# DIAGNijmegen/bodyct-dram-emph-subtype

Hardware: AMD Instinct MI355X
Metric: CT volumes/sec (train step, 1x128x256x256) (higher is better)
Workload: dtype f32; 1 GPU; BASELINE configs[1]: resnet18segcls train step (fwd+loss+bwd+Adam), batch 2/GPU, 1x128x256x256, fp32, inputs resident in HBM; global_batch=2, parallelism=dp1, hip_graph=False, streams=2

## Files before the change

### bodyct-dram-emph-subtype_amd/csrc/wino_gemm.hip

```cpp
#include <stdlib.h>
#include "wino_gemm.h"

namespace {

template <int MI, int NJ>
__device__ __forceinline__ void zero_acc(f32x16 (&acc)[MI][NJ]) {
#pragma unroll
  for (int mi = 0; mi < MI; ++mi)
#pragma unroll
    for (int nj = 0; nj < NJ; ++nj)
#pragma unroll
      for (int e = 0; e < 16; ++e) acc[mi][nj][e] = 0.f;
}


struct NnTile { const float* Ab; const float* Bb; float* Yb; int mt, nt; };
template <int NJ>
__device__ __forceinline__ NnTile nn_tile(const int idx, const float* A, const float* Bw, float* Y, const int N,
                                          const int K, const int m_tiles, const int n_tiles, const int nblk,
                                          const int npts) {
  constexpr int BN = 64 * NJ;
  const int L = xcd_remap(idx, nblk);
  NnTile t;
  t.nt = L % n_tiles;
  const int r0 = L / n_tiles;
  t.mt = r0 % m_tiles;
  const int xi = r0 / m_tiles;
  t.Ab = A + (((long)t.mt * npts + xi) * 256) * K;
  t.Bb = Bw + ((long)xi * N + (long)t.nt * BN) * K;
  t.Yb = Y + (((long)t.mt * npts + xi) * 256) * N + t.nt * BN;
  return t;
}

template <int NJ>
struct NnLane {
  int tid, lane, wave, li, lh, wm, wn, rsw, a_row, b_row;
  __device__ __forceinline__ NnLane() {
    tid = threadIdx.x;
    lane = tid & 63;
    wave = __builtin_amdgcn_readfirstlane(tid >> 6);
    li = lane & 31; lh = lane >> 5;
    wm = wave & 3; wn = wave >> 2;
    rsw = (li >> 1) & 7;
    a_row = (wm * 64 + li) * 32;
    b_row = 256 * 32 + (wn * NJ * 32 + li) * 32;
  }
};

template <int NJ>
struct NnDma {
  int wave, aoff[4], boff[NJ];
  __device__ __forceinline__ NnDma(const int lane, const int wave_, const int K) : wave(wave_) {
    const int sub = lane >> 3, pslot = lane & 7;
    const int s_even = pslot ^ (lane >> 4), s_odd = s_even ^ 4;
#pragma unroll
    for (int j = 0; j < 4; ++j) aoff[j] = (32 * wave + 8 * j + sub) * K + ((j & 1) ? s_odd : s_even) * 4;
#pragma unroll
    for (int jj = 0; jj < NJ; ++jj) {
      const int nrow = 8 * NJ * wave + 8 * jj + sub;
      boff[jj] = nrow * K + (pslot ^ ((nrow >> 1) & 7)) * 4;
    }
  }
  __device__ __forceinline__ void issue(const float* Ab, const float* Bb, const int it, float* stage) const {
    float* as = stage + 32 * wave * 32;
    float* bs = stage + 256 * 32 + 8 * NJ * wave * 32;
    const float* ag = Ab + it * 32;
    const float* bg = Bb + it * 32;
#pragma unroll
    for (int j = 0; j < 4; ++j)
      __builtin_amdgcn_global_load_lds((const __attribute__((address_space(1))) void*)(ag + aoff[j]),
                                       (__attribute__((address_space(3))) void*)(as + j * 8 * 32), 16, 0, 0);
#pragma unroll
    for (int jj = 0; jj < NJ; ++jj)
      __builtin_amdgcn_global_load_lds((const __attribute__((address_space(1))) void*)(bg + boff[jj]),
                                       (__attribute__((address_space(3))) void*)(bs + jj * 8 * 32), 16, 0, 0);
  }
};

template <int NJ>
__device__ __forceinline__ void nn_kgroups(const float* st, const NnLane<NJ>& ln, f32x16 (&acc)[2][NJ]) {
  f32x4 a0[2], a1[2], bf[2][NJ];
  auto frag = [&](int gk, int buf) __attribute__((always_inline)) {
    const int so = ((2 * gk + ln.lh) ^ ln.rsw) * 4;
    a0[buf] = *reinterpret_cast<const f32x4*>(st + ln.a_row + so);
    a1[buf] = *reinterpret_cast<const f32x4*>(st + ln.a_row + 32 * 32 + so);
#pragma unroll
    for (int nj = 0; nj < NJ; ++nj) bf[buf][nj] = *reinterpret_cast<const f32x4*>(st + ln.b_row + nj * 32 * 32 + so);
  };
  frag(0, 0);
#pragma unroll
  for (int gk = 0; gk < 4; ++gk) {
    if (gk + 1 < 4) frag(gk + 1, (gk + 1) & 1);
#pragma unroll
    for (int e = 0; e < 4; ++e) {
#pragma unroll
      for (int nj = 0; nj < NJ; ++nj) {
        acc[0][nj] = __builtin_amdgcn_mfma_f32_32x32x2f32(a0[gk & 1][e], bf[gk & 1][nj][e], acc[0][nj], 0, 0, 0);
        acc[1][nj] = __builtin_amdgcn_mfma_f32_32x32x2f32(a1[gk & 1][e], bf[gk & 1][nj][e], acc[1][nj], 0, 0, 0);
      }
    }
    if (gk + 1 < 4) __builtin_amdgcn_sched_group_barrier(0x100, 2 + NJ, 0);
    __builtin_amdgcn_sched_group_barrier(0x008, 8 * NJ, 0);
    __builtin_amdgcn_sched_barrier(0);
  }
}

template <int NJ>
__global__ __launch_bounds__(512) void wino_gemm_nn_kernel(const float* __restrict__ A, const float* __restrict__ Bw,
                                                           float* __restrict__ Y, const int Mpad, const int N,
                                                           const int K, const int m_tiles, const int n_tiles,
                                                           const int nblk, const int npts, const GemmEpilogue ep) {
  constexpr int STAGE = (256 + 64 * NJ) * 32;
  __shared__ __attribute__((aligned(1024))) float lds[2 * STAGE];
  const NnLane<NJ> ln;
  const NnTile t = nn_tile<NJ>(blockIdx.x, A, Bw, Y, N, K, m_tiles, n_tiles, nblk, npts);
  const NnDma<NJ> dma(ln.lane, ln.wave, K);
  const int niter = K / 32;
  f32x16 acc[2][NJ];
  zero_acc(acc);

  dma.issue(t.Ab, t.Bb, 0, lds);
  for (int it = 0; it < niter; ++it) {
    __syncthreads();
    if (it + 1 < niter) dma.issue(t.Ab, t.Bb, it + 1, lds + ((it + 1) & 1) * STAGE);
    nn_kgroups<NJ>(lds + (it & 1) * STAGE, ln, acc);
  }

  constexpr int BN = 64 * NJ;
  const bool fused = ep.bias || ep.add || ep.stats;
  constexpr int CW = NJ >= 2 ? 64 : 32;
  constexpr int NR = NJ >= 2 ? NJ / 2 : 1;
  constexpr int P = CW + 8;
  constexpr int Q = CW / 4;
  __syncthreads();
  float* reg = lds + ln.wave * (32 * P);
  const int cq = ln.lane % Q, rs = ln.lane / Q;
  float s1[NR][4], s2[NR][4];
#pragma unroll
  for (int cr = 0; cr < NR; ++cr)
#pragma unroll
    for (int j = 0; j < 4; ++j) { s1[cr][j] = 0.f; s2[cr][j] = 0.f; }
#pragma unroll
  for (int cr = 0; cr < NR; ++cr) {
    const int col = t.nt * BN + ln.wn * NJ * 32 + cr * CW + 4 * cq;
    f32x4 bv = {0.f, 0.f, 0.f, 0.f};
    if (ep.bias) bv = *reinterpret_cast<const f32x4*>(ep.bias + col);
#pragma unroll
    for (int mi = 0; mi < 2; ++mi) {
#pragma unroll
      for (int e = 0; e < 16; ++e)
#pragma unroll
        for (int j = 0; j < CW / 32; ++j)
          reg[((e & 3) + 8 * (e >> 2) + 4 * ln.lh) * P + j * 32 + ln.li] = acc[mi][cr * (CW / 32) + j][e];
#pragma unroll
      for (int r = 0; r < 32 / (64 / Q); ++r) {
        const int row = r * (64 / Q) + rs;
        f32x4 v = *reinterpret_cast<const f32x4*>(reg + row * P + 4 * cq);
        float* o = t.Yb + (long)(ln.wm * 64 + mi * 32 + row) * N + ln.wn * NJ * 32 + cr * CW + 4 * cq;
        if (fused) {
          v += bv;
          if (ep.add) {
            const long oo = o - Y;
            const f32x4 av = *reinterpret_cast<const f32x4*>(ep.add + oo);
            if (ep.gate) {
              const f32x4 gv = *reinterpret_cast<const f32x4*>(ep.gate + oo);
#pragma unroll
              for (int j = 0; j < 4; ++j) v[j] += gv[j] > 0.f ? av[j] : 0.f;
            } else {
              v += av;
            }
          }
#pragma unroll
          for (int j = 0; j < 4; ++j) { s1[cr][j] += v[j]; s2[cr][j] += v[j] * v[j]; }
        }
        *reinterpret_cast<f32x4*>(o) = v;
      }
    }
  }
  if (ep.stats) {
#pragma unroll
    for (int cr = 0; cr < NR; ++cr)
#pragma unroll
      for (int j = 0; j < 4; ++j)
#pragma unroll
        for (int o = Q; o < 64; o <<= 1) {
          s1[cr][j] += __shfl_xor(s1[cr][j], o, 64);
          s2[cr][j] += __shfl_xor(s2[cr][j], o, 64);
        }
    __syncthreads();
    float* red = lds;
    if (rs == 0) {
#pragma unroll
      for (int cr = 0; cr < NR; ++cr)
#pragma unroll
        for (int j = 0; j < 4; ++j) {
          red[(ln.wave * 2 + 0) * 32 * NJ + cr * CW + 4 * cq + j] = s1[cr][j];
          red[(ln.wave * 2 + 1) * 32 * NJ + cr * CW + 4 * cq + j] = s2[cr][j];
        }
    }
    __syncthreads();
    if (ln.tid < 2 * BN) {
      const int which = ln.tid / BN, cc = ln.tid - which * BN;
      const int cwn = cc / (32 * NJ), c2 = cc - cwn * 32 * NJ;
      float v = 0.f;
#pragma unroll
      for (int w = 0; w < 4; ++w) v += red[((cwn * 4 + w) * 2 + which) * 32 * NJ + c2];
      ep.stats[((long)t.mt * 2 + which) * N + t.nt * BN + cc] = v;
    }
  }
}

template <int NJ>
__global__ __launch_bounds__(512) void wino_gemm_nn_pers_kernel(const float* __restrict__ A, const float* __restrict__ Bw,
                                                                float* __restrict__ Y, const int Mpad, const int N,
                                                                const int K, const int m_tiles, const int n_tiles,
                                                                const int nblk, const int npts, const GemmEpilogue ep) {
  constexpr int STAGE = (256 + 64 * NJ) * 32;
  __shared__ __attribute__((aligned(1024))) float s0[STAGE];
  __shared__ __attribute__((aligned(1024))) float s1[STAGE + (NJ == 1 ? 1024 : 0)];
  const NnLane<NJ> ln;
  const NnDma<NJ> dma(ln.lane, ln.wave, K);
  constexpr int BN = 64 * NJ;
  const int niter = K / 32;
  const bool fused = ep.bias || ep.add || ep.stats;
  f32x16 acc[2][NJ];

  int idx = blockIdx.x;
  NnTile cur = nn_tile<NJ>(idx, A, Bw, Y, N, K, m_tiles, n_tiles, nblk, npts);
  dma.issue(cur.Ab, cur.Bb, 0, s0);
  for (;;) {
    const int nxt = idx + gridDim.x;
    const bool more = nxt < nblk;
    NnTile nx = cur;
    if (more) nx = nn_tile<NJ>(nxt, A, Bw, Y, N, K, m_tiles, n_tiles, nblk, npts);
    zero_acc(acc);
    for (int it = 0; it < niter; it += 2) {
      __syncthreads();
      dma.issue(cur.Ab, cur.Bb, it + 1, s1);
      nn_kgroups<NJ>(s0, ln, acc);
      __syncthreads();
      if (it + 2 < niter) dma.issue(cur.Ab, cur.Bb, it + 2, s0);
      else if (more) dma.issue(nx.Ab, nx.Bb, 0, s0);
      nn_kgroups<NJ>(s1, ln, acc);
    }

    constexpr int CW = NJ >= 2 ? 64 : 32;
    constexpr int NR = NJ >= 2 ? NJ / 2 : 1;
    constexpr int P = CW + 8;
    constexpr int Q = CW / 4;
    __syncthreads();
    float* reg = s1 + ln.wave * (16 * P);
    const int cq = ln.lane % Q, rs = ln.lane / Q;
    float s1v[NR][4], s2v[NR][4];
#pragma unroll
    for (int cr = 0; cr < NR; ++cr)
#pragma unroll
      for (int j = 0; j < 4; ++j) { s1v[cr][j] = 0.f; s2v[cr][j] = 0.f; }
#pragma unroll
    for (int cr = 0; cr < NR; ++cr) {
      const int col = cur.nt * BN + ln.wn * NJ * 32 + cr * CW + 4 * cq;
      f32x4 bv = {0.f, 0.f, 0.f, 0.f};
      if (ep.bias) bv = *reinterpret_cast<const f32x4*>(ep.bias + col);
#pragma unroll
      for (int mi = 0; mi < 2; ++mi) {
#pragma unroll
        for (int h = 0; h < 2; ++h) {
#pragma unroll
          for (int e = 8 * h; e < 8 * h + 8; ++e)
#pragma unroll
            for (int j = 0; j < CW / 32; ++j)
              reg[((e & 3) + 8 * ((e >> 2) & 1) + 4 * ln.lh) * P + j * 32 + ln.li] = acc[mi][cr * (CW / 32) + j][e];
#pragma unroll
          for (int r = 0; r < 16 / (64 / Q); ++r) {
            const int row = r * (64 / Q) + rs;
            f32x4 v = *reinterpret_cast<const f32x4*>(reg + row * P + 4 * cq);
            float* o = cur.Yb + (long)(ln.wm * 64 + mi * 32 + 16 * h + row) * N + ln.wn * NJ * 32 + cr * CW + 4 * cq;
            if (fused) {
              v += bv;
              if (ep.add) {
                const long oo = o - Y;
                const f32x4 av = *reinterpret_cast<const f32x4*>(ep.add + oo);
                if (ep.gate) {
                  const f32x4 gv = *reinterpret_cast<const f32x4*>(ep.gate + oo);
#pragma unroll
                  for (int j = 0; j < 4; ++j) v[j] += gv[j] > 0.f ? av[j] : 0.f;
                } else {
                  v += av;
                }
              }
#pragma unroll
              for (int j = 0; j < 4; ++j) { s1v[cr][j] += v[j]; s2v[cr][j] += v[j] * v[j]; }
            }
            *reinterpret_cast<f32x4*>(o) = v;
          }
        }
      }
    }
    if (ep.stats) {
#pragma unroll
      for (int cr = 0; cr < NR; ++cr)
#pragma unroll
        for (int j = 0; j < 4; ++j)
#pragma unroll
          for (int o = Q; o < 64; o <<= 1) {
            s1v[cr][j] += __shfl_xor(s1v[cr][j], o, 64);
            s2v[cr][j] += __shfl_xor(s2v[cr][j], o, 64);
          }
      __syncthreads();
      float* red = s1;
      if (rs == 0) {
#pragma unroll
        for (int cr = 0; cr < NR; ++cr)
#pragma unroll
          for (int j = 0; j < 4; ++j) {
            red[(ln.wave * 2 + 0) * 32 * NJ + cr * CW + 4 * cq + j] = s1v[cr][j];
            red[(ln.wave * 2 + 1) * 32 * NJ + cr * CW + 4 * cq + j] = s2v[cr][j];
          }
      }
      __syncthreads();
      if (ln.tid < 2 * BN) {
        const int which = ln.tid / BN, cc = ln.tid - which * BN;
        const int cwn = cc / (32 * NJ), c2 = cc - cwn * 32 * NJ;
        float v = 0.f;
#pragma unroll
        for (int w = 0; w < 4; ++w) v += red[((cwn * 4 + w) * 2 + which) * 32 * NJ + c2];
        ep.stats[((long)cur.mt * 2 + which) * N + cur.nt * BN + cc] = v;
      }
    }
    if (!more) break;
    idx = nxt;
    cur = nx;
  }
}
#ifndef DRAM_STREAM_NT
#define DRAM_STREAM_NT 2
#endif
template <int NJ, int KT, int S, bool DB = false, int KH = 1>
__global__ __launch_bounds__(256, DB ? 2 : 1) void wino_gemm_nn_stream_kernel(const float* __restrict__ A,
                                                                    const float* __restrict__ Bw, float* __restrict__ Y,
                                                                    const int npts, const int m64, const int per_wg,
                                                                    const int total) {
  constexpr int N = 64 * NJ;
  constexpr int STG = 64 * KT;
  constexpr int SPR = KT / 4;
  constexpr int RPI = 64 / SPR;
  constexpr int IPW = 64 / RPI / 4;
  constexpr int BPW = N / RPI / 4;
  constexpr int KG = KT / 8;
  constexpr int P = DB ? 40 : 32 * NJ + 8;
  constexpr int KS = KT * KH;
  static_assert(S == 3 || S == 4, "ring depth");
  static_assert(KH == 1 || (KH == 2 && DB && S == 3), "k halves: direct-B form, three stages");
  __shared__ __attribute__((aligned(1024))) float st0[STG], st1[STG], st2[STG], st3[S == 4 ? STG : 64];
  __shared__ __attribute__((aligned(1024))) float bt[DB ? 64 : N * KT];
  __shared__ __attribute__((aligned(16))) float turn[4 * 32 * P];

  const int tid = threadIdx.x, lane = tid & 63;
  const int wave = __builtin_amdgcn_readfirstlane(tid >> 6);
  const int li = lane & 31, lh = lane >> 5;
  const int i0 = blockIdx.x * per_wg;
  const int n = (i0 + per_wg <= total ? per_wg : total - i0);
  if (n <= 0) return;

  int aoff[IPW], boff[BPW];
#pragma unroll
  for (int j = 0; j < IPW; ++j) {
    const int row = RPI * (wave + 4 * j) + lane / SPR, ph = lane % SPR;
    aoff[j] = row * KS + ((ph & ~15) | ((ph ^ row) & 15)) * 4;
  }
#pragma unroll
  for (int j = 0; j < BPW; ++j) {
    const int row = RPI * (wave + 4 * j) + lane / SPR, ph = lane % SPR;
    boff[j] = row * KT + ((ph & ~15) | ((ph ^ row) & 15)) * 4;
  }
  auto a_src = [&](int item) __attribute__((always_inline)) {
    const int ti = item / KH, h = item - ti * KH;
    const int xi = ti / m64, t = ti - xi * m64;
    return A + (((long)(t >> 2) * npts + xi) * 256 + (t & 3) * 64) * KS + h * KT;
  };
  auto issue_a = [&](int item, float* stage) __attribute__((always_inline)) {
    const float* src = a_src(item);
#pragma unroll
    for (int j = 0; j < IPW; ++j)
      __builtin_amdgcn_global_load_lds((const __attribute__((address_space(1))) void*)(src + aoff[j]),
                                       (__attribute__((address_space(3))) void*)(stage + (wave + 4 * j) * 256), 16, 0,
                                       DRAM_STREAM_NT);
  };
  auto stage_of = [&](int k) __attribute__((always_inline)) -> float* {
    return k == 0 ? st0 : (k == 1 ? st1 : (k == 2 ? st2 : st3));
  };

  const int r0 = 32 * (wave & 1), c0 = 32 * NJ * (wave >> 1);
  const int arow = r0 + li;
  f32x4 bfr[NJ][KG * KH];
  auto load_b = [&](int xi) __attribute__((always_inline)) {
    if (DB) {
      const float* srcd = Bw + (long)xi * N * KS;
#pragma unroll
      for (int nj = 0; nj < NJ; ++nj)
#pragma unroll
        for (int kg = 0; kg < KG * KH; ++kg)
          bfr[nj][kg] = *reinterpret_cast<const f32x4*>(srcd + (c0 + nj * 32 + li) * KS + (2 * kg + lh) * 4);
      __builtin_amdgcn_s_waitcnt(0x0F70);
      asm volatile("" ::: "memory");
      return;
    }
    __syncthreads();
    const float* src = Bw + (long)xi * N * KT;
#pragma unroll
    for (int j = 0; j < BPW; ++j)
      __builtin_amdgcn_global_load_lds((const __attribute__((address_space(1))) void*)(src + boff[j]),
                                       (__attribute__((address_space(3))) void*)(bt + (wave + 4 * j) * 256), 16, 0, 0);
    __builtin_amdgcn_s_waitcnt(0x0F70);
    asm volatile("" ::: "memory");
    __syncthreads();
#pragma unroll
    for (int nj = 0; nj < NJ; ++nj) {
      const int brow = c0 + nj * 32 + li;
#pragma unroll
      for (int kg = 0; kg < KG; ++kg) {
        const int sl = 2 * kg + lh;
        bfr[nj][kg] = *reinterpret_cast<const f32x4*>(bt + brow * KT + ((sl & ~15) | ((sl ^ brow) & 15)) * 4);
      }
    }
  };

  int xi_cur = i0 / KH / m64;
#pragma unroll
  for (int k = 0; k < S - 1; ++k)
    if (k < n) issue_a(i0 + k, stage_of(k));
  load_b(xi_cur);

  float* reg = turn + wave * (32 * P);
  constexpr int Q = 8 * NJ;
  const int cq = lane % Q, rs = lane / Q;

  constexpr int U = S * KH;
  f32x16 acc[NJ];
  for (int itb = 0; itb < n; itb += U) {
#pragma unroll
    for (int k = 0; k < U; ++k) {
      const int it = itb + k;
      const int h = k % KH;
      if (it < n) {
        const int item = i0 + it;
        const int ti = item / KH;
        const int xi = ti / m64, t = ti - xi * m64;
        if (h == 0 && xi != xi_cur) {
          xi_cur = xi;
          load_b(xi);
        }
        if (it + S - 2 < n) __builtin_amdgcn_s_waitcnt(0x0F70 | ((IPW * (S - 2)) & 15) | (((IPW * (S - 2)) >> 4) << 14));
        else __builtin_amdgcn_s_waitcnt(0x0F70);
        asm volatile("" ::: "memory");
        __builtin_amdgcn_s_barrier();
        if (it + S - 1 < n) issue_a(item + S - 1, stage_of((k + S - 1) % S));
        const float* stg = stage_of(k % S);
        if (h == 0) {
#pragma unroll
          for (int nj = 0; nj < NJ; ++nj)
#pragma unroll
            for (int e = 0; e < 16; ++e) acc[nj][e] = 0.f;
        }
#pragma unroll
        for (int kg = 0; kg < KG; ++kg) {
          const int sl = 2 * kg + lh;
          const f32x4 af = *reinterpret_cast<const f32x4*>(stg + arow * KT + ((sl & ~15) | ((sl ^ arow) & 15)) * 4);
#pragma unroll
          for (int e = 0; e < 4; ++e)
#pragma unroll
            for (int nj = 0; nj < NJ; ++nj)
              acc[nj] = __builtin_amdgcn_mfma_f32_32x32x2f32(af[e], bfr[nj][h * KG + kg][e], acc[nj], 0, 0, 0);
        }
        if (h != KH - 1) continue;
        float* yb = Y + (((long)(t >> 2) * npts + xi) * 256 + (t & 3) * 64 + r0) * N + c0;
        if (DB) {
          const int cq8 = lane & 7, rs8 = lane >> 3;
#pragma unroll
          for (int nj = 0; nj < NJ; ++nj) {
#pragma unroll
            for (int e = 0; e < 16; ++e) reg[((e & 3) + 8 * (e >> 2) + 4 * lh) * P + li] = acc[nj][e];
#pragma unroll
            for (int r = 0; r < 4; ++r) {
              const int row = r * 8 + rs8;
              *reinterpret_cast<f32x4*>(yb + (long)row * N + nj * 32 + 4 * cq8) =
                  *reinterpret_cast<const f32x4*>(reg + row * P + 4 * cq8);
            }
          }
        } else {
#pragma unroll
          for (int e = 0; e < 16; ++e)
#pragma unroll
            for (int nj = 0; nj < NJ; ++nj) reg[((e & 3) + 8 * (e >> 2) + 4 * lh) * P + nj * 32 + li] = acc[nj][e];
#pragma unroll
          for (int r = 0; r < Q / 2; ++r) {
            const int row = r * (64 / Q) + rs;
            *reinterpret_cast<f32x4*>(yb + (long)row * N + 4 * cq) = *reinterpret_cast<const f32x4*>(reg + row * P + 4 * cq);
          }
        }
      }
    }
  }
}

typedef __bf16 bf16x8 __attribute__((ext_vector_type(8)));

template <int NJ, int NT>
__global__ __launch_bounds__(512) void wino_gemm_nn_bf16_kernel(const float* __restrict__ A, const float* __restrict__ Bw,
                                                                float* __restrict__ Y, const int Mpad, const int N,
                                                                const int K, const int m_tiles, const int n_tiles,
                                                                const int nblk, const int npts) {
  constexpr int STAGE = (256 + 64 * NJ) * 32;
  __shared__ __attribute__((aligned(1024))) float lds[2 * STAGE];
  const int tid = threadIdx.x;
  const int lane = tid & 63;
  const int wave = __builtin_amdgcn_readfirstlane(tid >> 6);
  const NnTile t = nn_tile<NJ>(blockIdx.x, A, Bw, Y, N, K, m_tiles, n_tiles, nblk, npts);
  const NnDma<NJ> dma(lane, wave, K);
  const int niter = K / 32;
  f32x16 acc[2][NJ];
  zero_acc(acc);

  const int li = lane & 31, lh = lane >> 5;
  const int wm = wave & 3, wn = wave >> 2;
  const int rsw = (li >> 1) & 7;
  const int a_row = (wm * 64 + li) * 32;
  const int b_row = 256 * 32 + (wn * NJ * 32 + li) * 32;

  dma.issue(t.Ab, t.Bb, 0, lds);
  for (int it = 0; it < niter; ++it) {
    __syncthreads();
    if (it + 1 < niter) dma.issue(t.Ab, t.Bb, it + 1, lds + ((it + 1) & 1) * STAGE);
    const float* st = lds + (it & 1) * STAGE;
#pragma unroll
    for (int j = 0; j < 2; ++j) {
      const int sh = ((2 * j + lh) ^ rsw) * 4, sl = ((4 + 2 * j + lh) ^ rsw) * 4;
      bf16x8 ah[2], al[2], bh[NJ], bl[NJ];
#pragma unroll
      for (int mi = 0; mi < 2; ++mi) {
        ah[mi] = *reinterpret_cast<const bf16x8*>(st + a_row + mi * 32 * 32 + sh);
        if (NT > 1) al[mi] = *reinterpret_cast<const bf16x8*>(st + a_row + mi * 32 * 32 + sl);
      }
#pragma unroll
      for (int nj = 0; nj < NJ; ++nj) {
        bh[nj] = *reinterpret_cast<const bf16x8*>(st + b_row + nj * 32 * 32 + sh);
        if (NT > 1) bl[nj] = *reinterpret_cast<const bf16x8*>(st + b_row + nj * 32 * 32 + sl);
      }
#pragma unroll
      for (int nj = 0; nj < NJ; ++nj)
#pragma unroll
        for (int mi = 0; mi < 2; ++mi) {
          if (NT > 1) {
            acc[mi][nj] = __builtin_amdgcn_mfma_f32_32x32x16_bf16(al[mi], bh[nj], acc[mi][nj], 0, 0, 0);
            acc[mi][nj] = __builtin_amdgcn_mfma_f32_32x32x16_bf16(ah[mi], bl[nj], acc[mi][nj], 0, 0, 0);
          }
          acc[mi][nj] = __builtin_amdgcn_mfma_f32_32x32x16_bf16(ah[mi], bh[nj], acc[mi][nj], 0, 0, 0);
        }
    }
  }

#pragma unroll
  for (int mi = 0; mi < 2; ++mi)
#pragma unroll
    for (int e = 0; e < 16; ++e) {
      const int row = wm * 64 + mi * 32 + (e & 3) + 8 * (e >> 2) + 4 * lh;
      float* o = t.Yb + (long)row * N + wn * NJ * 32 + li;
#pragma unroll
      for (int nj = 0; nj < NJ; ++nj) o[nj * 32] = acc[mi][nj][e];
    }
}

struct TnTile {
  int nt, mt, split, xi;
  int t0, t1;
  __device__ __forceinline__ long row(const int it, const int npts) const {
    const int tt = t0 + it * 32;
    return ((long)(tt >> 8) * npts + xi) * 256 + (tt & 255);
  }
};
__device__ __forceinline__ TnTile tn_item(int L, const int m_tiles, const int n_tiles, const int nsplit, const int kper,
                                          const int Tpad) {
  TnTile t;
  t.nt = L % n_tiles; L /= n_tiles;
  t.mt = L % m_tiles; L /= m_tiles;
  t.split = L % nsplit;
  t.xi = L / nsplit;
  t.t0 = t.split * kper;
  t.t1 = (t.t0 + kper < Tpad) ? t.t0 + kper : Tpad;
  return t;
}
__device__ __forceinline__ TnTile tn_tile(const int bid, const int nblk, const int m_tiles, const int n_tiles,
                                          const int nsplit, const int kper, const int Tpad) {
  return tn_item(xcd_remap(bid, nblk), m_tiles, n_tiles, nsplit, kper, Tpad);
}
template <int WMW, int MI, int NJ>
__global__ __launch_bounds__(512) void wino_gemm_tn_kernel(const float* __restrict__ Ah, const float* __restrict__ Bh,
                                                           float* __restrict__ slab, const int Tpad, const int M,
                                                           const int N, const int m_tiles, const int n_tiles,
                                                           const int nsplit, const int kper, const int nblk,
                                                           const int npts) {
  constexpr int WNW = 8 / WMW;
  constexpr int BM = WMW * 32 * MI, BN = WNW * 32 * NJ;
  static_assert(BM % 64 == 0 && BM <= 256 && BN % 64 == 0 && BN <= 256, "one DMA piece = 256 floats");
  constexpr int STAGE = 32 * (BM + BN);
  constexpr int AQ = BM / 4, ARPP = 64 / AQ, APW = BM / 64;
  constexpr int BQ = BN / 4, BRPP = 64 / BQ, BPW = BN / 64;
  __shared__ __attribute__((aligned(1024))) float lds[2 * STAGE];

  const int tid = threadIdx.x;
  const int lane = tid & 63;
  const int wave = __builtin_amdgcn_readfirstlane(tid >> 6);
  const TnTile t = tn_tile(blockIdx.x, nblk, m_tiles, n_tiles, nsplit, kper, Tpad);
  int bcol = t.nt * BN + (lane % BQ) * 4;
  if (bcol > N - 4) bcol = N - 4;
  const float* Ab = Ah + (long)(lane / AQ) * M + t.mt * BM + (lane % AQ) * 4;
  const float* Bb = Bh + (long)(lane / BQ) * N + bcol;

  auto issue = [&](int it, int stage) __attribute__((always_inline)) {
    float* as = lds + stage * STAGE;
    float* bs = as + 32 * BM;
    const long row = t.row(it, npts);
    const float* ag = Ab + row * M;
    const float* bg = Bb + row * N;
#pragma unroll
    for (int j = 0; j < APW; ++j) {
      const int p = APW * wave + j;
      __builtin_amdgcn_global_load_lds((const __attribute__((address_space(1))) void*)(ag + (long)(p * ARPP) * M),
                                       (__attribute__((address_space(3))) void*)(as + p * 256), 16, 0, 0);
    }
#pragma unroll
    for (int jj = 0; jj < BPW; ++jj) {
      const int p = BPW * wave + jj;
      __builtin_amdgcn_global_load_lds((const __attribute__((address_space(1))) void*)(bg + (long)(p * BRPP) * N),
                                       (__attribute__((address_space(3))) void*)(bs + p * 256), 16, 0, 0);
    }
  };
// ... 272 lines not shown
      else __builtin_amdgcn_s_waitcnt(0x0F70);
      asm volatile("" ::: "memory");
      __builtin_amdgcn_s_barrier();
      if (full || it + S - 1 < n) issue(it + S - 1, a_of((k + S - 1) % S), b_of((k + S - 1) % S));
      const float* as = a_of(k) + wm * 32 + li;
      const float* bs = b_of(k) + wn * 64 + li;
#pragma unroll
      for (int kk = 0; kk < R / 2; ++kk) {
        const int kr = 2 * kk + lh;
        const float af = as[kr * M], b0 = bs[kr * N], b1 = bs[kr * N + 32];
        acc[0] = __builtin_amdgcn_mfma_f32_32x32x2f32(af, b0, acc[0], 0, 0, 0);
        acc[1] = __builtin_amdgcn_mfma_f32_32x32x2f32(af, b1, acc[1], 0, 0, 0);
      }
    };
    int itb = 0;
    for (; itb + 2 * S - 2 < n; itb += S) {
#pragma unroll
      for (int k = 0; k < S; ++k) stage(k, itb + k, true);
    }
    for (; itb < n; itb += S) {
#pragma unroll
      for (int k = 0; k < S; ++k)
        if (itb + k < n) stage(k, itb + k, false);
    }

    float* sb = slab + (((long)split * npts + xi) * M) * N;
#pragma unroll
    for (int e = 0; e < 16; ++e) {
      const int row = wm * 32 + (e & 3) + 8 * (e >> 2) + 4 * lh;
      float* o = sb + (long)row * N + wn * 64 + li;
      o[0] = acc[0][e];
      o[32] = acc[1][e];
    }
  }
}

typedef short s16x4 __attribute__((ext_vector_type(4)));
typedef short s16x8 __attribute__((ext_vector_type(8)));

template <int WMW, int MI, int NJ, int NT>
__global__ __launch_bounds__(512) void wino_gemm_tn_bf16_kernel(const float* __restrict__ Ah, const float* __restrict__ Bh,
                                                                float* __restrict__ slab, const int Tpad, const int M,
                                                                const int N, const int m_tiles, const int n_tiles,
                                                                const int nsplit, const int kper, const int nblk,
                                                                const int npts) {
  constexpr int WNW = 8 / WMW;
  constexpr int BM = WMW * 32 * MI, BN = WNW * 32 * NJ;
  static_assert(BM % 64 == 0 && BM <= 256 && BN % 64 == 0 && BN <= 256, "one DMA piece = 256 floats");
  constexpr int STAGE = 32 * (BM + BN);
  constexpr int AQ = BM / 4, ARPP = 64 / AQ, APW = BM / 64;
  constexpr int BQ = BN / 4, BRPP = 64 / BQ, BPW = BN / 64;
  __shared__ __attribute__((aligned(1024))) float lds[2 * STAGE];

  const int tid = threadIdx.x;
  const int lane = tid & 63;
  const int wave = __builtin_amdgcn_readfirstlane(tid >> 6);
  const TnTile t = tn_tile(blockIdx.x, nblk, m_tiles, n_tiles, nsplit, kper, Tpad);

  int acol[APW], bcol[BPW];
#pragma unroll
  for (int j = 0; j < APW; ++j) {
    const int r3 = (j * ARPP + lane / AQ) & 3, slot = lane % AQ;
    acol[j] = t.mt * BM + ((((slot >> 2) ^ r3) << 2) | (slot & 3)) * 4;
  }
#pragma unroll
  for (int j = 0; j < BPW; ++j) {
    const int r3 = (j * BRPP + lane / BQ) & 3, slot = lane % BQ;
    int c = t.nt * BN + ((((slot >> 2) ^ r3) << 2) | (slot & 3)) * 4;
    bcol[j] = c > N - 4 ? N - 4 : c;
  }
  const float* Ab = Ah + (long)(lane / AQ) * M;
  const float* Bb = Bh + (long)(lane / BQ) * N;

  auto issue = [&](int it, int stage) __attribute__((always_inline)) {
    float* as = lds + stage * STAGE;
    float* bs = as + 32 * BM;
    const long row = t.row(it, npts);
    const float* ag = Ab + row * M;
    const float* bg = Bb + row * N;
#pragma unroll
    for (int j = 0; j < APW; ++j) {
      const int p = APW * wave + j;
      __builtin_amdgcn_global_load_lds((const __attribute__((address_space(1))) void*)(ag + (long)(p * ARPP) * M + acol[j]),
                                       (__attribute__((address_space(3))) void*)(as + p * 256), 16, 0, 0);
    }
#pragma unroll
    for (int jj = 0; jj < BPW; ++jj) {
      const int p = BPW * wave + jj;
      __builtin_amdgcn_global_load_lds((const __attribute__((address_space(1))) void*)(bg + (long)(p * BRPP) * N + bcol[jj]),
                                       (__attribute__((address_space(3))) void*)(bs + p * 256), 16, 0, 0);
    }
  };

  f32x16 acc[MI][NJ];
  zero_acc(acc);

  const int li = lane & 31, lh = lane >> 5;
  const int wm = wave % WMW, wn = wave / WMW;
  const int niter = (t.t1 - t.t0) / 32;

  const int g4 = lane >> 4, q = (lane >> 2) & 3, p4 = lane & 3;
  const int rrow = (g4 >> 1) * 8 + q;
  const int cbyte = (g4 & 1) * 32 + p4 * 8;
  int a_hi[MI], a_lo[MI], b_hi[NJ], b_lo[NJ];
#pragma unroll
  for (int mi = 0; mi < MI; ++mi) {
    const int ch = 2 * (wm * MI + mi);
    a_hi[mi] = rrow * BM * 4 + ((ch ^ q) * 64) + cbyte;
    a_lo[mi] = rrow * BM * 4 + (((ch + 1) ^ q) * 64) + cbyte;
  }
#pragma unroll
  for (int nj = 0; nj < NJ; ++nj) {
    const int ch = 2 * (wn * NJ + nj);
    b_hi[nj] = 32 * BM * 4 + rrow * BN * 4 + ((ch ^ q) * 64) + cbyte;
    b_lo[nj] = 32 * BM * 4 + rrow * BN * 4 + (((ch + 1) ^ q) * 64) + cbyte;
  }
  auto frag = [&](const char* st, int off, int rstride) __attribute__((always_inline)) {
    const s16x4 r0 = __builtin_amdgcn_ds_read_tr16_b64_v4i16((__attribute__((address_space(3))) s16x4*)(st + off));
    const s16x4 r1 =
        __builtin_amdgcn_ds_read_tr16_b64_v4i16((__attribute__((address_space(3))) s16x4*)(st + off + 4 * rstride));
    return __builtin_bit_cast(bf16x8, __builtin_shufflevector(r0, r1, 0, 1, 2, 3, 4, 5, 6, 7));
  };

  if (niter > 0) issue(0, 0);
  for (int it = 0; it < niter; ++it) {
    __syncthreads();
    if (it + 1 < niter) issue(it + 1, (it + 1) & 1);
    const char* st = reinterpret_cast<const char*>(lds + (it & 1) * STAGE);
#pragma unroll
    for (int s16 = 0; s16 < 2; ++s16) {
      bf16x8 ah[MI], al[MI], bh[NJ], bl[NJ];
#pragma unroll
      for (int mi = 0; mi < MI; ++mi) {
        ah[mi] = frag(st, a_hi[mi] + s16 * 16 * BM * 4, BM * 4);
        if (NT > 1) al[mi] = frag(st, a_lo[mi] + s16 * 16 * BM * 4, BM * 4);
      }
#pragma unroll
      for (int nj = 0; nj < NJ; ++nj) {
        bh[nj] = frag(st, b_hi[nj] + s16 * 16 * BN * 4, BN * 4);
        if (NT > 1) bl[nj] = frag(st, b_lo[nj] + s16 * 16 * BN * 4, BN * 4);
      }
#pragma unroll
      for (int nj = 0; nj < NJ; ++nj)
#pragma unroll
        for (int mi = 0; mi < MI; ++mi) {
          if (NT > 1) {
            acc[mi][nj] = __builtin_amdgcn_mfma_f32_32x32x16_bf16(al[mi], bh[nj], acc[mi][nj], 0, 0, 0);
            acc[mi][nj] = __builtin_amdgcn_mfma_f32_32x32x16_bf16(ah[mi], bl[nj], acc[mi][nj], 0, 0, 0);
          }
          acc[mi][nj] = __builtin_amdgcn_mfma_f32_32x32x16_bf16(ah[mi], bh[nj], acc[mi][nj], 0, 0, 0);
        }
    }
  }

  float* sb = slab + (((long)t.split * npts + t.xi) * M + t.mt * BM) * N + t.nt * BN;
#pragma unroll
  for (int mi = 0; mi < MI; ++mi)
#pragma unroll
    for (int e = 0; e < 16; ++e) {
      const int row = wm * 32 * MI + mi * 32 + (e & 3) + 8 * (e >> 2) + 4 * lh;
      float* o = sb + (long)row * N + wn * 32 * NJ + li;
#pragma unroll
      for (int nj = 0; nj < NJ; ++nj)
        if (t.nt * BN + wn * 32 * NJ + nj * 32 + li < N) o[nj * 32] = acc[mi][nj][e];
    }
}

__global__ __launch_bounds__(256) void slab_sum_kernel(const float* __restrict__ slab, float* __restrict__ out, const long n,
                                                       const int nsplit) {
  __shared__ float part[4][64];
  const int r = threadIdx.x & 63, kg = threadIdx.x >> 6;
  for (long i0 = blockIdx.x * 64L; i0 < n; i0 += (long)gridDim.x * 64L) {
    const long i = i0 + r;
    const bool live = i < n;
    float p[8];
#pragma unroll
    for (int j = 0; j < 8; ++j) p[j] = 0.f;
    if (live) {
      int k = kg;
      for (; k + 28 < nsplit; k += 32) {
#pragma unroll
        for (int j = 0; j < 8; ++j) p[j] += slab[(long)(k + 4 * j) * n + i];
      }
      for (int j = 0; k < nsplit; k += 4, ++j) p[j] += slab[(long)k * n + i];
    }
    part[kg][r] = ((p[0] + p[1]) + (p[2] + p[3])) + ((p[4] + p[5]) + (p[6] + p[7]));
    __syncthreads();
    if (kg == 0 && live) out[i] = (part[0][r] + part[1][r]) + (part[2][r] + part[3][r]);
    __syncthreads();
  }
}
}


bool plan_tn(const DramConvDesc* d, const WinoGeom& g, TnPlan& p) {
  const int M = d->Cout, N = d->Cin;
  p.bm = M % 256 == 0 ? 256 : (M % 128 == 0 ? 128 : 64);
  const int ncand = p.bm == 256 ? 3 : 2;
  const int cand[3] = {256, 128, 64};
  p.bn = 0;
  int best_pad = 1 << 30;
  for (int i = 0; i < ncand; ++i) {
    const int padded = (N + cand[i] - 1) / cand[i] * cand[i];
    if (padded * 100 <= N * 113) { p.bn = cand[i]; break; }
    if (padded < best_pad) { best_pad = padded; p.bn = cand[i]; }
  }
  p.m_tiles = M / p.bm;
  p.n_tiles = (N + p.bn - 1) / p.bn;
  if (p.bn >= 128 && (p.bn > 128 || p.bm == 256)) {
    const long w1 = (long)g.npts * p.m_tiles * p.n_tiles;
    const int hb = p.bn / 2, hn = (N + hb - 1) / hb;
    const long w2 = (long)g.npts * p.m_tiles * hn;
    if (w1 >= 512 && (double)((w2 + 255) / 256) * 0.5 * 1.03 < (double)((w1 + 255) / 256)) {
      p.bn = hb;
      p.n_tiles = hn;
    }
  }
  const int base = g.npts * p.m_tiles * p.n_tiles;
  const int k32 = g.Tpad / 32;
  int ns = 1;
  while (base * ns < (g.npts == 1 ? 256 : 512) && ns * 2 <= k32 / 4 && ns < (g.npts == 1 ? 256 : 16)) ns *= 2;
  p.nsplit = ns;
  p.kper = ((k32 + ns - 1) / ns) * 32;
  return true;
}

int run_nn(const float* A, const float* U, float* Y, const WinoGeom& g, int N, int K, hipStream_t s,
           const GemmEpilogue ep, const int math, const bool alone) {
  const int m_tiles = g.Tpad / 256;
  int nj = 1;
  double best = 1e30;
  for (int c = 4; c >= 1; c >>= 1) {
    if (N % (64 * c) != 0) continue;
    const long wgs = (long)g.npts * m_tiles * (N / (64 * c));
    const double cost = (double)((wgs + 255) / 256) * c * (c == 4 ? 1.0 : (c == 2 ? 1.03 : 1.10));
    if (cost < best) { best = cost; nj = c; }
  }
  const int n_tiles = N / (64 * nj);
  const int nblk = g.npts * m_tiles * n_tiles;
  DramProf prof(DRAM_FAM_WINO_GEMM_NN, nj, 2.0 * g.npts * (double)g.Tpad * N * K,
                4.0 * g.npts * ((double)g.Tpad * (K + N) + (double)N * K), s,
                g.npts > 1 ? 2.0 * g.B * g.D * g.H * g.W * (double)N * K * 27.0 : -1.0);
  if (math) {
#define WNB(NJ_, NT_)                                                                                                  \
  hipLaunchKernelGGL((wino_gemm_nn_bf16_kernel<NJ_, NT_>), dim3(nblk), dim3(512), 0, s, A, U, Y, g.Tpad, N, K, m_tiles, \
                     n_tiles, nblk, g.npts)
    if (math == 1) { if (nj == 4) WNB(4, 3); else if (nj == 2) WNB(2, 3); else WNB(1, 3); }
    else { if (nj == 4) WNB(4, 1); else if (nj == 2) WNB(2, 1); else WNB(1, 1); }
#undef WNB
    DRAM_LAUNCH_CHECK();
    return DRAM_OK;
  }
#define WNN(NJ_)                                                                                                   \
  hipLaunchKernelGGL((wino_gemm_nn_kernel<NJ_>), dim3(nblk), dim3(512), 0, s, A, U, Y, g.Tpad, N, K, m_tiles, n_tiles, \
                     nblk, g.npts, ep)
  const char* se = tune_env("DRAM_NN_STREAM");
  const int stream_on = se ? atoi(se) : 1;
  const bool fused = ep.bias || ep.add || ep.gate || ep.stats;
  if (stream_on && !fused && g.npts > 1 && g.Tpad % 256 == 0 &&
      ((N == 64 && (K == 128 || K == 64)) || (N == 128 && K == 64))) {
    const int m64 = g.Tpad / 64;
    const long total = (long)g.npts * m64;
    if (total < (1L << 31) && (total >= 4096 || stream_on == 2)) {
      const int wgs = stream_on == 2 ? 8 : 256;
      const int per_wg = (int)((total + wgs - 1) / wgs);
      const int grid = (int)((total + per_wg - 1) / per_wg);
#define WNS(NJ_, KT_, S_)                                                                                          \
  hipLaunchKernelGGL((wino_gemm_nn_stream_kernel<NJ_, KT_, S_>), dim3(grid), dim3(256), 0, s, A, U, Y, g.npts, m64, \
                     per_wg, (int)total)
      const char* sde = tune_env("DRAM_NN_STREAM_DB");
      const int sdb = sde ? atoi(sde) : (alone ? 7 : 0);
      const int wgs2 = stream_on == 2 ? 8 : 512;
      const int per2 = (int)((total + wgs2 - 1) / wgs2);
      const int grid2 = (int)((total + per2 - 1) / per2);
      if (N == 64 && K == 128 && (sdb & 4)) {
        const long total2 = 2 * total;
        if (total2 < (1L << 31)) {
          const int perk = 2 * (int)((total + wgs2 - 1) / wgs2);
          const int gridk = (int)((total2 + perk - 1) / perk);
          hipLaunchKernelGGL((wino_gemm_nn_stream_kernel<1, 64, 3, true, 2>), dim3(gridk), dim3(256), 0, s, A, U, Y, g.npts,
                             m64, perk, (int)total2);
        } else WNS(1, 128, 3);
      }
      else if (N == 64 && K == 128) WNS(1, 128, 3);
      else if (N == 64 && (sdb & 1))
        hipLaunchKernelGGL((wino_gemm_nn_stream_kernel<1, 64, 3, true>), dim3(grid2), dim3(256), 0, s, A, U, Y, g.npts, m64,
                           per2, (int)total);
      else if (N == 128 && (sdb & 2))
        hipLaunchKernelGGL((wino_gemm_nn_stream_kernel<2, 64, 3, true>), dim3(grid2), dim3(256), 0, s, A, U, Y, g.npts, m64,
                           per2, (int)total);
      else if (N == 64) WNS(1, 64, 4);
      else WNS(2, 64, 4);
#undef WNS
      DRAM_LAUNCH_CHECK();
      return DRAM_OK;
    }
  }
  const char* pe = tune_env("DRAM_NN_PERSIST");
  const int persist = pe ? atoi(pe) : 1;
  if (persist && !fused && nj <= 2 && (K / 32) % 2 == 0) {
    const int rounds = (nblk + 255) / 256;
    int grid = ((nblk + rounds - 1) / rounds + 7) / 8 * 8;
    if (grid > 256) grid = 256;
    if (grid > nblk) grid = nblk;
#define WNP(NJ_)                                                                                                   \
  hipLaunchKernelGGL((wino_gemm_nn_pers_kernel<NJ_>), dim3(grid), dim3(512), 0, s, A, U, Y, g.Tpad, N, K, m_tiles, \
                     n_tiles, nblk, g.npts, ep)
    if (nj == 2) WNP(2);
    else WNP(1);
#undef WNP
    DRAM_LAUNCH_CHECK();
    return DRAM_OK;
  }
  if (nj == 4) WNN(4);
  else if (nj == 2) WNN(2);
  else WNN(1);
#undef WNN
  DRAM_LAUNCH_CHECK();
  return DRAM_OK;
}

int run_tn(const float* Ah, const float* Bh, float* slab, const WinoGeom& g, const TnPlan& p, const int M, const int N,
           const int math, hipStream_t s) {
  const int nblk = g.npts * p.nsplit * p.m_tiles * p.n_tiles;
  DramProf prof(DRAM_FAM_WINO_GEMM_TN, p.bm * 1000 + p.bn, 2.0 * g.npts * (double)g.Tpad * M * N,
                4.0 * g.npts * ((double)g.Tpad * (M + N) + (double)p.nsplit * M * N), s,
                g.npts > 1 ? 2.0 * g.B * g.D * g.H * g.W * (double)M * N * 27.0 : -1.0);
  auto launch = [&](auto kernel) {
    hipLaunchKernelGGL(kernel, dim3(nblk), dim3(512), 0, s, Ah, Bh, slab, g.Tpad, M, N, p.m_tiles, p.n_tiles, p.nsplit,
                       p.kper, nblk, g.npts);
  };
#define WTN(WM_, MI_, NJ_)                                             \
  launch(math == 1   ? wino_gemm_tn_bf16_kernel<WM_, MI_, NJ_, 3>      \
         : math == 2 ? wino_gemm_tn_bf16_kernel<WM_, MI_, NJ_, 1>      \
                     : wino_gemm_tn_kernel<WM_, MI_, NJ_>)
  const char* te = tune_env("DRAM_NN_STREAM");
  const int tn_stream = te ? atoi(te) : 1;
  if (math == 0 && tn_stream) {
    const bool t64 = g.npts > 1 && M == 64 && N == 64 && p.kper % 64 == 0 && g.Tpad % 64 == 0;
    if (g.npts > 1 && M == 64 && N == 128 && p.bm == 64 && p.bn == 128) {
      const int nchains = g.npts * p.nsplit;
      const int grid = tn_stream == 2 && nchains > 8 ? 8 : nchains;
      hipLaunchKernelGGL((wino_gemm_tn_stream_kernel<3>), dim3(grid), dim3(256), 0, s, Ah, Bh, slab, g.Tpad, p.nsplit, p.kper,
                         nchains, g.npts);
      DRAM_LAUNCH_CHECK();
      return DRAM_OK;
    }
    const int niter = p.kper / 32;
    const bool whole = niter % 2 == 0 && (long)p.kper * p.nsplit == g.Tpad;
    if (!t64 && whole && (tn_stream == 2 || (g.npts > 1 && niter <= 4))) {
      const int slots = 256 * (p.bm + p.bn <= 256 ? 2 : 1);
      const int rounds = (nblk + slots - 1) / slots;
      int grid = ((nblk + rounds - 1) / rounds + 7) / 8 * 8;
      if (grid > slots) grid = slots;
      if (tn_stream == 2) grid = 8;
      if (grid > nblk) grid = nblk;
      const int per_wg = (nblk + grid - 1) / grid;
      grid = (nblk + per_wg - 1) / per_wg;
      if (per_wg > 1 || tn_stream == 2) {
#define WTP(WM_, MI_, NJ_)                                                                                              \
  hipLaunchKernelGGL((wino_gemm_tn_pers_kernel<WM_, MI_, NJ_>), dim3(grid), dim3(512), 0, s, Ah, Bh, slab, g.Tpad, M, N, \
                     p.m_tiles, p.n_tiles, p.nsplit, p.kper, nblk, g.npts, per_wg)
        if (p.bm == 256 && p.bn == 256) WTP(4, 2, 4);
        else if (p.bm == 256 && p.bn == 128) WTP(4, 2, 2);
        else if (p.bm == 256 && p.bn == 64) WTP(4, 2, 1);
        else if (p.bm == 128 && p.bn == 256) WTP(2, 2, 2);
        else if (p.bm == 128 && p.bn == 128) WTP(2, 2, 1);
        else if (p.bm == 64 && p.bn == 256) WTP(2, 1, 2);
        else if (p.bm == 64 && p.bn == 128) WTP(2, 1, 1);
        else return DRAM_ERR_UNSUPPORTED;
#undef WTP
        DRAM_LAUNCH_CHECK();
        return DRAM_OK;
      }
    }
  }
  if (math == 0 && g.npts > 1 && M == 64 && N == 64 && p.kper % 64 == 0 && g.Tpad % 64 == 0)
    hipLaunchKernelGGL(wino_gemm_tn64_kernel, dim3(g.npts * p.nsplit), dim3(512), 0, s, Ah, Bh, slab, g.Tpad, p.nsplit,
                       p.kper, g.npts * p.nsplit, g.npts);
  else if (p.bm == 256 && p.bn == 256) WTN(4, 2, 4);
  else if (p.bm == 256 && p.bn == 128) WTN(4, 2, 2);
  else if (p.bm == 256 && p.bn == 64) WTN(4, 2, 1);
  else if (p.bm == 128 && p.bn == 256) WTN(2, 2, 2);
  else if (p.bm == 128 && p.bn == 128) WTN(2, 2, 1);
  else if (p.bm == 64 && p.bn == 256) WTN(2, 1, 2);
  else if (p.bm == 64 && p.bn == 128) WTN(2, 1, 1);
  else return DRAM_ERR_UNSUPPORTED;
#undef WTN
  DRAM_LAUNCH_CHECK();
  return DRAM_OK;
}

namespace {
bool c1_ok(const DramConvDesc* d) {
  if (!d || d->k != 1 || d->stride != 1 || d->pad != 0) return false;
  if (d->B < 1 || d->D < 1 || d->H < 1 || d->W < 1) return false;
  if (d->Do != d->D || d->Ho != d->H || d->Wo != d->W) return false;
  if (d->Cin < 64 || d->Cout < 64 || d->Cin % 64 != 0 || d->Cout % 64 != 0) return false;
  const long long M = (long long)d->B * d->D * d->H * d->W;
  const long long cmax = d->Cin > d->Cout ? d->Cin : d->Cout;
  return M % 256 == 0 && M * cmax < (1LL << 31);
}
WinoGeom c1_geom(const DramConvDesc* d) {
  WinoGeom g{};
  g.B = d->B; g.D = d->D; g.H = d->H; g.W = d->W; g.d = 1;
  g.nz = g.ny = g.nx = 1;
  g.npts = 1;
  g.T = g.Tpad = d->B * d->D * d->H * d->W;
  return g;
}
}

extern "C" int dram_conv1x1_applicable(const DramConvDesc* d) { return c1_ok(d) ? 1 : 0; }

extern "C" int dram_conv1x1_num_stat_rows(const DramConvDesc* d) {
  if (!c1_ok(d)) return DRAM_ERR_UNSUPPORTED;
  return c1_geom(d).Tpad / 256;
}

extern "C" int dram_conv1x1_fwd(const float* x, const float* w2d, const float* bias, float* y, float* stats_partial,
                                const DramConvDesc* d, dram_stream_t stream) {
  if (!x || !w2d || !y) return DRAM_ERR_BAD_ARG;
  if (!c1_ok(d)) return DRAM_ERR_UNSUPPORTED;
  return run_nn(x, w2d, y, c1_geom(d), d->Cout, d->Cin, (hipStream_t)stream,
                GemmEpilogue{bias, nullptr, nullptr, stats_partial});
}

extern "C" int dram_conv1x1_bwd_data(const float* dy, const float* wt, float* dx, const float* add, const float* gate,
                                     const DramConvDesc* d, dram_stream_t stream) {
  if (!dy || !wt || !dx || (gate && !add)) return DRAM_ERR_BAD_ARG;
  if (!c1_ok(d)) return DRAM_ERR_UNSUPPORTED;
  return run_nn(dy, wt, dx, c1_geom(d), d->Cin, d->Cout, (hipStream_t)stream, GemmEpilogue{nullptr, add, gate, nullptr});
}

extern "C" size_t dram_conv1x1_bwd_weight_workspace(const DramConvDesc* d) {
  if (!c1_ok(d)) return 0;
  TnPlan p;
  plan_tn(d, c1_geom(d), p);
  return (size_t)p.nsplit * d->Cout * d->Cin * sizeof(float);
}

extern "C" int dram_conv1x1_bwd_weight(const float* x, const float* dy, float* dw, const DramConvDesc* d, void* workspace,
                                       size_t workspace_bytes, dram_stream_t stream) {
  if (!x || !dy || !dw) return DRAM_ERR_BAD_ARG;
  if (!c1_ok(d)) return DRAM_ERR_UNSUPPORTED;
  const WinoGeom g = c1_geom(d);
  TnPlan p;
  plan_tn(d, g, p);
  const size_t need = (size_t)p.nsplit * d->Cout * d->Cin * sizeof(float);
  if (p.nsplit > 1 && (!workspace || workspace_bytes < need)) return DRAM_ERR_WORKSPACE;
  hipStream_t s = (hipStream_t)stream;
  float* slab = p.nsplit > 1 ? (float*)workspace : dw;
  const int rc = run_tn(dy, x, slab, g, p, d->Cout, d->Cin, 0, s);
  if (rc != DRAM_OK) return rc;
  if (p.nsplit > 1) {
    const long n = (long)d->Cout * d->Cin;
    const int grid = (int)((n + 63) / 64 > 4096 ? 4096 : (n + 63) / 64);
    DramProf prof(DRAM_FAM_WINO_WGRAD_OUT, 0, 0.0, 4.0 * (double)n * (p.nsplit + 1), s);
    hipLaunchKernelGGL(slab_sum_kernel, dim3(grid), dim3(256), 0, s, slab, dw, n, p.nsplit);
    DRAM_LAUNCH_CHECK();
  }
  return DRAM_OK;
}
```

Measured before the change: 56.00 volumes/sec.

## Overlap persistent NN GEMM epilogue stores with next tile's MFMA main loop

Adds a persistent Winograd NN GEMM kernel that keeps two accumulator sets and drains the previous tile's results through a per-wave LDS transpose buffer, interleaved into the first k-groups of the next tile using sched_group_barrier. The aim is to hide epilogue store latency behind MFMA work instead of stalling at the end of each tile. It becomes the default for the persistent, non-fused path (persist=3 restores the old kernel). It drops the fused stats epilogue from this path and doubles accumulator registers, which risks register pressure. There is also a debug grid=7 option.

```diff
diff --git a/bodyct-dram-emph-subtype_amd/csrc/wino_gemm.hip b/bodyct-dram-emph-subtype_amd/csrc/wino_gemm.hip
--- a/bodyct-dram-emph-subtype_amd/csrc/wino_gemm.hip
+++ b/bodyct-dram-emph-subtype_amd/csrc/wino_gemm.hip
@@ -1,4 +1,5 @@
 #include <stdlib.h>
+#include <type_traits>
 #include "wino_gemm.h"
 
 namespace {
@@ -332,6 +333,214 @@
     cur = nx;
   }
 }
+
+template <int NJ>
+struct NnTurn {
+  static constexpr int CW = 32 * NJ;
+  static constexpr int P = CW + 8;
+  static constexpr int Q = CW / 4;
+  static constexpr int RPR = 64 / Q;
+  static constexpr int NRD = 16 / RPR;
+  static constexpr int NWR = 8 * NJ;
+  float* reg;
+  float* po;
+  int N, cq, rs;
+  template <int T>
+  __device__ __forceinline__ void write(const NnLane<NJ>& ln, const f32x16 (&prev)[2][NJ]) const {
+#pragma unroll
+    for (int e = 8 * (T & 1); e < 8 * (T & 1) + 8; ++e)
+#pragma unroll
+      for (int j = 0; j < NJ; ++j)
+        reg[((e & 3) + 8 * ((e >> 2) & 1) + 4 * ln.lh) * P + j * 32 + ln.li] = prev[T >> 1][j][e];
+  }
+  __device__ __forceinline__ void read(f32x4 (&v)[NRD]) const {
+#pragma unroll
+    for (int r = 0; r < NRD; ++r) v[r] = *reinterpret_cast<const f32x4*>(reg + (r * RPR + rs) * P + 4 * cq);
+  }
+  template <int T>
+  __device__ __forceinline__ void store(const f32x4 (&v)[NRD]) const {
+#pragma unroll
+    for (int r = 0; r < NRD; ++r)
+      *reinterpret_cast<f32x4*>(po + (long)((T >> 1) * 32 + (T & 1) * 16 + r * RPR) * N) = v[r];
+  }
+  __device__ __forceinline__ void all(const NnLane<NJ>& ln, const f32x16 (&prev)[2][NJ]) const {
+    f32x4 v[NRD];
+    write<0>(ln, prev); read(v); store<0>(v);
+    write<1>(ln, prev); read(v); store<1>(v);
+    write<2>(ln, prev); read(v); store<2>(v);
+    write<3>(ln, prev); read(v); store<3>(v);
+  }
+};
+
+template <int NJ, int T0, int NT>
+__device__ __forceinline__ void nn_kgroups_drain(const float* st, const NnLane<NJ>& ln, f32x16 (&acc)[2][NJ],
+                                                 const f32x16 (&prev)[2][NJ], const NnTurn<NJ>& tr) {
+  using TR = NnTurn<NJ>;
+  f32x4 a0[2], a1[2], bf[2][NJ];
+  f32x4 va[TR::NRD], vb[TR::NRD];
+  auto frag = [&](int gk, int buf) __attribute__((always_inline)) {
+    const int so = ((2 * gk + ln.lh) ^ ln.rsw) * 4;
+    a0[buf] = *reinterpret_cast<const f32x4*>(st + ln.a_row + so);
+    a1[buf] = *reinterpret_cast<const f32x4*>(st + ln.a_row + 32 * 32 + so);
+#pragma unroll
+    for (int nj = 0; nj < NJ; ++nj) bf[buf][nj] = *reinterpret_cast<const f32x4*>(st + ln.b_row + nj * 32 * 32 + so);
+  };
+  frag(0, 0);
+  auto region = [&](auto gkc) __attribute__((always_inline)) {
+    constexpr int gk = decltype(gkc)::value;
+    if (gk + 1 < 4) frag(gk + 1, (gk + 1) & 1);
+    if constexpr (NT == 1) {
+      if (gk == 0) { tr.template write<T0>(ln, prev); tr.read(va); }
+      if (gk == 1) tr.template store<T0>(va);
+    } else {
+      if (gk == 0) tr.template write<T0>(ln, prev);
+      if (gk == 1) { tr.read(va); tr.template write<T0 + NT - 1>(ln, prev); }
+      if (gk == 2) { tr.template store<T0>(va); tr.read(vb); }
+      if (gk == 3) tr.template store<T0 + NT - 1>(vb);
+    }
+#pragma unroll
+    for (int e = 0; e < 4; ++e) {
+#pragma unroll
+      for (int nj = 0; nj < NJ; ++nj) {
+        acc[0][nj] = __builtin_amdgcn_mfma_f32_32x32x2f32(a0[gk & 1][e], bf[gk & 1][nj][e], acc[0][nj], 0, 0, 0);
+        acc[1][nj] = __builtin_amdgcn_mfma_f32_32x32x2f32(a1[gk & 1][e], bf[gk & 1][nj][e], acc[1][nj], 0, 0, 0);
+      }
+    }
+    constexpr bool rd = NT == 2 && (gk == 1 || gk == 2);
+    constexpr bool wr = (gk == 0) || (gk == 1 && NT == 2);
+    constexpr bool stg = NT == 2 ? (gk == 2 || gk == 3) : gk == 1;
+    constexpr int nrd = (gk + 1 < 4 ? 2 + NJ : 0) + (rd ? TR::NRD : 0);
+    if constexpr (nrd > 0) __builtin_amdgcn_sched_group_barrier(0x100, nrd, 0);
+    if constexpr (wr && NT == 1) {
+#pragma unroll
+      for (int i = 0; i < 4; ++i) {
+        __builtin_amdgcn_sched_group_barrier(0x008, 1, 0);
+        __builtin_amdgcn_sched_group_barrier(0x200, 2, 0);
+      }
+      __builtin_amdgcn_sched_group_barrier(0x008, 2, 0);
+      __builtin_amdgcn_sched_group_barrier(0x100, TR::NRD, 0);
+      __builtin_amdgcn_sched_group_barrier(0x008, 8 * NJ - 6, 0);
+    } else if constexpr (wr) {
+#pragma unroll
+      for (int i = 0; i < TR::NWR; ++i) {
+        __builtin_amdgcn_sched_group_barrier(0x008, 1, 0);
+        __builtin_amdgcn_sched_group_barrier(0x200, 1, 0);
+      }
+    } else if constexpr (stg) {
+#pragma unroll
+      for (int i = 0; i < TR::NRD; ++i) {
+        __builtin_amdgcn_sched_group_barrier(0x008, 1, 0);
+        __builtin_amdgcn_sched_group_barrier(0x040, 1, 0);
+      }
+      __builtin_amdgcn_sched_group_barrier(0x008, 8 * NJ - TR::NRD, 0);
+    } else {
+      __builtin_amdgcn_sched_group_barrier(0x008, 8 * NJ, 0);
+    }
+    __builtin_amdgcn_sched_barrier(0);
+  };
+  region(std::integral_constant<int, 0>{});
+  region(std::integral_constant<int, 1>{});
+  region(std::integral_constant<int, 2>{});
+  region(std::integral_constant<int, 3>{});
+}
+
+template <int NJ>
+__device__ __forceinline__ void nn_drain_tile(float* s0, float* s1, const NnLane<NJ>& ln, const NnDma<NJ>& dma,
+                                              const NnTile& cur, const NnTile& nx, const bool more, const int niter,
+                                              f32x16 (&acc)[2][NJ], const f32x16 (&prev)[2][NJ], const bool drain,
+                                              const NnTurn<NJ>& tr) {
+  zero_acc(acc);
+  int it = 0;
+  if (drain) {
+    if (niter == 2) {
+      __syncthreads();
+      dma.issue(cur.Ab, cur.Bb, 1, s1);
+      nn_kgroups_drain<NJ, 0, 2>(s0, ln, acc, prev, tr);
+      __syncthreads();
+      if (more) dma.issue(nx.Ab, nx.Bb, 0, s0);
+      nn_kgroups_drain<NJ, 2, 2>(s1, ln, acc, prev, tr);
+      it = 2;
+    } else {
+      __syncthreads();
+      dma.issue(cur.Ab, cur.Bb, 1, s1);
+      nn_kgroups_drain<NJ, 0, 1>(s0, ln, acc, prev, tr);
+      __syncthreads();
+      dma.issue(cur.Ab, cur.Bb, 2, s0);
+      nn_kgroups_drain<NJ, 1, 1>(s1, ln, acc, prev, tr);
+      __syncthreads();
+      dma.issue(cur.Ab, cur.Bb, 3, s1);
+      nn_kgroups_drain<NJ, 2, 1>(s0, ln, acc, prev, tr);
+      __syncthreads();
+      if (4 < niter) dma.issue(cur.Ab, cur.Bb, 4, s0);
+      else if (more) dma.issue(nx.Ab, nx.Bb, 0, s0);
+      nn_kgroups_drain<NJ, 3, 1>(s1, ln, acc, prev, tr);
+      it = 4;
+    }
+  }
+  for (; it < niter; it += 2) {
+    __syncthreads();
+    dma.issue(cur.Ab, cur.Bb, it + 1, s1);
+    nn_kgroups<NJ>(s0, ln, acc);
+    __syncthreads();
+    if (it + 2 < niter) dma.issue(cur.Ab, cur.Bb, it + 2, s0);
+    else if (more) dma.issue(nx.Ab, nx.Bb, 0, s0);
+    nn_kgroups<NJ>(s1, ln, acc);
+  }
+}
+
+template <int NJ>
+__global__ __launch_bounds__(512) void wino_gemm_nn_drain_kernel(const float* __restrict__ A, const float* __restrict__ Bw,
+                                                                 float* __restrict__ Y, const int N, const int K,
+                                                                 const int m_tiles, const int n_tiles, const int nblk,
+                                                                 const int npts) {
+  static_assert(NJ == 1 || NJ == 2, "one column round per turn");
+  constexpr int STAGE = (256 + 64 * NJ) * 32;
+  __shared__ __attribute__((aligned(1024))) float s0[STAGE];
+  __shared__ __attribute__((aligned(1024))) float s1[STAGE];
+  __shared__ __attribute__((aligned(16))) float turn[8 * 16 * NnTurn<NJ>::P];
+  const NnLane<NJ> ln;
+  const NnDma<NJ> dma(ln.lane, ln.wave, K);
+  const int niter = K / 32;
+  f32x16 acc0[2][NJ], acc1[2][NJ];
+  NnTurn<NJ> tr;
+  tr.reg = turn + ln.wave * (16 * NnTurn<NJ>::P);
+  tr.N = N;
+  tr.cq = ln.lane % NnTurn<NJ>::Q;
+  tr.rs = ln.lane / NnTurn<NJ>::Q;
+  tr.po = Y;
+  const long lane_off = (long)(ln.wm * 64 + tr.rs) * N + ln.wn * NJ * 32 + 4 * tr.cq;
+
+  int idx = blockIdx.x;
+  NnTile cur = nn_tile<NJ>(idx, A, Bw, Y, N, K, m_tiles, n_tiles, nblk, npts);
+  dma.issue(cur.Ab, cur.Bb, 0, s0);
+  bool pend = false;
+  for (;;) {
+    {
+      const int nxt = idx + gridDim.x;
+      const bool more = nxt < nblk;
+      NnTile nx = cur;
+      if (more) nx = nn_tile<NJ>(nxt, A, Bw, Y, N, K, m_tiles, n_tiles, nblk, npts);
+      nn_drain_tile<NJ>(s0, s1, ln, dma, cur, nx, more, niter, acc0, acc1, pend, tr);
+      tr.po = cur.Yb + lane_off;
+      if (!more) { tr.all(ln, acc0); break; }
+      idx = nxt;
+      cur = nx;
+    }
+    {
+      const int nxt = idx + gridDim.x;
+      const bool more = nxt < nblk;
+      NnTile nx = cur;
+      if (more) nx = nn_tile<NJ>(nxt, A, Bw, Y, N, K, m_tiles, n_tiles, nblk, npts);
+      nn_drain_tile<NJ>(s0, s1, ln, dma, cur, nx, more, niter, acc1, acc0, true, tr);
+      tr.po = cur.Yb + lane_off;
+      if (!more) { tr.all(ln, acc1); break; }
+      idx = nxt;
+      cur = nx;
+      pend = true;
+    }
+  }
+}
+
 #ifndef DRAM_STREAM_NT
 #define DRAM_STREAM_NT 2
 #endif
@@ -1210,8 +1419,19 @@
     const int rounds = (nblk + 255) / 256;
     int grid = ((nblk + rounds - 1) / rounds + 7) / 8 * 8;
     if (grid > 256) grid = 256;
+    if (persist == 2) grid = 7;
     if (grid > nblk) grid = nblk;
-#define WNP(NJ_)                                                                                                   \
+    if (persist != 3) {
+      if (nj == 2)
+        hipLaunchKernelGGL((wino_gemm_nn_drain_kernel<2>), dim3(grid), dim3(512), 0, s, A, U, Y, N, K, m_tiles, n_tiles, nblk,
+                           g.npts);
+      else
+        hipLaunchKernelGGL((wino_gemm_nn_drain_kernel<1>), dim3(grid), dim3(512), 0, s, A, U, Y, N, K, m_tiles, n_tiles, nblk,
+                           g.npts);
+      DRAM_LAUNCH_CHECK();
+      return DRAM_OK;
+    }
+#define WNP(NJ_)                                                                                                  \
   hipLaunchKernelGGL((wino_gemm_nn_pers_kernel<NJ_>), dim3(grid), dim3(512), 0, s, A, U, Y, g.Tpad, N, K, m_tiles, \
                      n_tiles, nblk, g.npts, ep)
     if (nj == 2) WNP(2);
```

After: 55.96 volumes/sec. Within noise of the previous version (-0.1%).
